# xiaochuanle/hifimeth

Hardware: AMD Instinct MI355X
Metric: cytosine sites/sec (CpG+CHG+CHH) (higher is better)
Workload: dtype f16x3+f32acc

## Files before the change

### hifimeth_amd/csrc/hm_convs.h

```cpp
#pragma once
#include "hm_convh.h"

namespace hm {

struct WRegs {
    half8 w[12][4][2];
    float4 bz[4];
};

struct DenseRows {
    static constexpr bool DENSE = true;
    static constexpr int M = 1 << 30;
};
template <int LOUT, int ISS, int MSTR, int ROW0, int M_>
struct SiteRows {
    static constexpr bool DENSE = false;
    static constexpr int M = M_;
    template <class C>
    static __device__ __forceinline__ int off(int m) {
        const int mc = m < M ? m : M - 1, site = mc / LOUT, p = mc - site * LOUT;
        return site * ISS + (MSTR * p + ROW0) * C::IRS;
    }
};

template <int CIN_, int KT_, int IRS_, int DIL_, bool WLO_, bool XLO_, int KSTACK_, int XD_, int NTW_ = 2>
struct SCfg {
    static constexpr int CIN = CIN_, KT = KT_, IRS = IRS_, DIL = DIL_, KSTACK = KSTACK_, XD = XD_, NTW = NTW_;
    static constexpr bool WLO = WLO_ && KSTACK_ == 0, XLO = XLO_;
    static constexpr int KB = KT * CIN / 32;
    static constexpr int WSTR = KSTACK ? 64 : 128;
    static constexpr int NTERM = 1 + (XLO ? 1 : 0) + (WLO ? 1 : 0);
    static_assert(KB <= 12 && (KT * CIN) % 32 == 0 && (CIN % 32 == 0 || KSTACK > 0), "bad streaming conv geometry");
    static __device__ __forceinline__ int lane_off(int kb, int lk) {
        if constexpr (KSTACK > 0) {
            int t = 4 * kb + lk;
            t = t >= 2 * KSTACK ? 0 : t >= KSTACK ? t - KSTACK : t;
            return t * IRS;
        } else {
            const int kk = kb * 32, tap = kk / CIN;
            return tap * DIL * IRS + (kk - tap * CIN) + 8 * lk;
        }
    }
};

template <int I, int N, class F>
__device__ __forceinline__ void static_for(F&& f) {
    if constexpr (I < N) {
        f(std::integral_constant<int, I>{});
        static_for<I + 1, N>(f);
    }
}

template <class C, int K0, int K1>
__device__ __forceinline__ void sconv_load_w(const half_t* __restrict__ wfrag, int nt0, int lane, WRegs& W) {
    const half8* wp = reinterpret_cast<const half8*>(wfrag) + (size_t)nt0 * C::KB * C::WSTR + lane;
    static_for<K0, K1>([&](auto kb_) __attribute__((always_inline)) {
        constexpr int kb = decltype(kb_)::value;
#pragma unroll
        for (int j = 0; j < C::NTW; ++j) {
            W.w[kb][j][0] = wp[(size_t)(j * C::KB + kb) * C::WSTR];
            if (C::WLO) W.w[kb][j][1] = wp[(size_t)(j * C::KB + kb) * C::WSTR + 64];
        }
    });
}
template <class C>
__device__ __forceinline__ void sconv_load_bias(const float* __restrict__ bias, int nt0, int lane, WRegs& W) {
#pragma unroll
    for (int j = 0; j < C::NTW; ++j) W.bz[j] = *reinterpret_cast<const float4*>(bias + (nt0 + j) * 16 + 4 * (lane >> 4));
}

template <class C, class CN, class RM, int T0, int... GS>
struct SConvR {
    static constexpr int NG = sizeof...(GS);
    static constexpr int gs[NG] = {GS...};
    static constexpr int gmax() { int m = 0; for (int g = 0; g < NG; ++g) m = gs[g] > m ? gs[g] : m; return m; }
    static constexpr int gs_at(int g) { return g < NG ? gs[g < NG ? g : 0] : 0; }
    static constexpr int NTW = C::NTW;
    static constexpr int tile0(int g) { int t = T0; for (int i = 0; i < g; ++i) t += gs[i]; return t; }
    static constexpr int GMAX = gmax(), KB = C::KB, NB = NG * KB, XS = C::XD + 1;

    struct NoCopy {
        static constexpr int CS = 0, NWV = 4;
        const uint8_t* rows = nullptr;
        half_t* g = nullptr;
    };
    template <int J0 = 0, class Epi, class Copy = NoCopy>
    static __device__ __forceinline__ void run(const half_t* __restrict__ in_hi, const half_t* __restrict__ in_lo, WRegs& W,
                                               Epi epi, const half_t* __restrict__ wnext, const float* __restrict__ bnext,
                                               int nt0, int nt0n, Copy cp = Copy{}, RM rm = RM{}) {
        int tid = threadIdx.x;
        asm volatile("" : "+v"(tid));
        const int lane = tid & 63, li = lane & 15, lk = lane >> 4;
        const int a0 = li * C::IRS;
        constexpr int NTILES = tile0(NG) - T0;
        int aoff[RM::DENSE ? 1 : NTILES];
        if constexpr (!RM::DENSE) {
#pragma unroll
            for (int t = 0; t < NTILES; ++t) aoff[t] = rm.template off<C>((T0 + t) * 16 + li);
        }
        f32x4 acc[2][GMAX][NTW];
        half8 x[XS][GMAX][2];
        constexpr int CS = Copy::CS;
        static_assert(CS + 2 <= NB, "a copy slot per k-block");
        int crow[3];
        half8 cdat[2];
        const uint8_t* cpr = CS > 0 ? cp.rows + 2 * __builtin_amdgcn_readfirstlane(tid >> 6) + (lane >> 5) : nullptr;

        auto reads = [&](auto c_) __attribute__((always_inline)) {
            constexpr int c = decltype(c_)::value, g = c / KB, kb = c % KB;
            const int off = C::lane_off(kb, lk);
#pragma unroll
            for (int i = 0; i < gs[g]; ++i) {
                int o;
                if constexpr (RM::DENSE) o = a0 + off + (tile0(g) + i) * 16 * C::IRS;
                else o = aoff[RM::DENSE ? 0 : tile0(g) + i - T0] + off;
                x[c % XS][i][0] = *reinterpret_cast<const half8*>(in_hi + o);
                if (C::XLO) x[c % XS][i][1] = *reinterpret_cast<const half8*>(in_lo + o);
            }
        };
        static_for<0, (C::XD < NB ? C::XD : NB)>(reads);

        static_for<0, NB>([&](auto c_) __attribute__((always_inline)) {
            constexpr int c = decltype(c_)::value, g = c / KB, kb = c % KB, G = gs[g];
            if constexpr (kb == 0) {
#pragma unroll
                for (int i = 0; i < G; ++i)
#pragma unroll
                    for (int j = 0; j < NTW; ++j) acc[g & 1][i][j] = f32x4{W.bz[J0 + j].x, W.bz[J0 + j].y, W.bz[J0 + j].z, W.bz[J0 + j].w};
            }
            if constexpr (!std::is_void_v<CN> && g == NG - 1 && kb == 0)
                sconv_load_bias<std::conditional_t<std::is_void_v<CN>, C, CN>>(bnext, nt0n, lane, W);
            if constexpr (c + C::XD < NB) reads(std::integral_constant<int, c + C::XD>{});
#pragma unroll
            for (int pr = 0; pr < 3; ++pr) {
                if ((pr == 1 && !C::XLO) || (pr == 2 && !C::WLO)) continue;
#pragma unroll
                for (int i = 0; i < G; ++i)
#pragma unroll
                    for (int j = 0; j < NTW; ++j)
                        acc[g & 1][i][j] = __builtin_amdgcn_mfma_f32_16x16x32_f16(W.w[kb][J0 + j][pr == 2 ? 1 : 0], x[c % XS][i][pr == 1 ? 1 : 0],
                                                                                 acc[g & 1][i][j], 0, 0, 0);
            }
            constexpr int NA = g > 0 ? gs[g > 0 ? g - 1 : 0] * NTW : 0;
            constexpr int A0 = kb * NA / KB, A1 = (kb + 1) * NA / KB;
            if constexpr (g > 0) {
#pragma unroll
                for (int a = A0; a < A1; ++a) {
                    const int m = (tile0(g - 1) + a / NTW) * 16 + li;
                    if ((tile0(g - 1) + a / NTW + 1) * 16 <= RM::M || m < RM::M) epi(m, (nt0 + J0 + a % NTW) * 16 + 4 * lk, acc[(g - 1) & 1][a / NTW][a % NTW]);
                }
            }
            if constexpr (c >= 2 && c < CS + 2)
                *reinterpret_cast<half8*>(cp.g + (size_t)crow[(c - 2) % 3] * 256 + (lane & 31) * 8) = cdat[(c - 2) & 1];
            if constexpr (c >= 1 && c < CS + 1)
                cdat[(c - 1) & 1] = *reinterpret_cast<const half8*>(((lane & 16) ? in_lo : in_hi) + crow[(c - 1) % 3] * C::IRS + (lane & 15) * 8);
            if constexpr (c < CS) crow[c % 3] = cpr[c * 2 * Copy::NWV];
            if constexpr (!std::is_void_v<CN>) {
                using CNN = std::conditional_t<std::is_void_v<CN>, C, CN>;
                constexpr int NPN = CNN::WLO ? 2 : 1, EN = CNN::KB * CNN::NTW * NPN;
                auto is_free = [](int e) constexpr {
                    const int kb2 = e / (CNN::NTW * NPN), j2 = e / NPN % CNN::NTW, p2 = e % NPN;
                    return kb2 >= KB || j2 < J0 || j2 >= J0 + NTW || p2 >= (C::WLO ? 2 : 1);
                };
                constexpr int NFREE = [&]() constexpr { int n = 0; for (int e = 0; e < EN; ++e) n += is_free(e); return n; }();
                constexpr int NEARLY = NB - KB;
                const half8* wp = reinterpret_cast<const half8*>(wnext) + (size_t)nt0n * CNN::KB * CNN::WSTR + lane;
                static_for<0, EN>([&](auto e_) __attribute__((always_inline)) {
                    constexpr int e = decltype(e_)::value;
                    constexpr int kb2 = e / (CNN::NTW * NPN), j2 = e / NPN % CNN::NTW, p2 = e % NPN;
                    constexpr bool fr = is_free(e);
                    constexpr int rank = [&]() constexpr { int n = 0; for (int q = 0; q < e; ++q) n += is_free(q); return n; }();
                    constexpr bool now = fr ? (NEARLY > 0 ? (c < NEARLY && rank * NEARLY / (NFREE > 0 ? NFREE : 1) == c) : (c == NB - KB))
                                            : (g == NG - 1 && kb2 == kb);
                    if constexpr (now) W.w[kb2][j2][p2] = wp[(size_t)(j2 * CNN::KB + kb2) * CNN::WSTR + 64 * p2];
                });
            }
            {
                constexpr int ND = gs_at((c + C::XD) / KB) * (C::XLO ? 2 : 1);
                constexpr int NM = C::NTERM * G * NTW;
                constexpr int NR = NM > ND ? NM - ND : 1;
                constexpr int NV = g > 0 ? ((A1 - A0) * 24 + NR - 1) / NR : 0;
#pragma unroll
                for (int q = 0; q < (ND < NM ? ND : NM); ++q) {
                    __builtin_amdgcn_sched_group_barrier(0x008, 1, 0);
                    __builtin_amdgcn_sched_group_barrier(0x100, 1, 0);
                }
#pragma unroll
                for (int q = 0; q < NM - ND; ++q) {
                    __builtin_amdgcn_sched_group_barrier(0x008, 1, 0);
                    if (NV > 0) __builtin_amdgcn_sched_group_barrier(0x002, NV, 0);
                    if (NV > 0) __builtin_amdgcn_sched_group_barrier(0x200, 1, 0);
                    __builtin_amdgcn_sched_group_barrier(0x020, 1, 0);
                    if (c <= CS + 1) __builtin_amdgcn_sched_group_barrier(0x140, 1, 0);
                }
            }
            __builtin_amdgcn_sched_barrier(0);
        });
        {
            constexpr int g = NG - 1;
#pragma unroll
            for (int a = 0; a < gs[g] * NTW; ++a) {
                const int m = (tile0(g) + a / NTW) * 16 + li;
                if ((tile0(g) + a / NTW + 1) * 16 <= RM::M || m < RM::M) epi(m, (nt0 + J0 + a % NTW) * 16 + 4 * lk, acc[g & 1][a / NTW][a % NTW]);
            }
        }
    }
};

template <class C, class CN, int T0, int... GS>
using SConv = SConvR<C, CN, DenseRows, T0, GS...>;

}
```

### hifimeth_amd/csrc/hm_trunk3.hip

```cpp
#include "hm_convh.h"
#ifdef HM_TRUNK_STAMP
#include "hm_stamp.h"
namespace hm { __device__ unsigned long long g_trunk3_stamp[8][24]; }
extern "C" int hm_debug_trunk3_stamps(unsigned long long* out, int reset) {
    if (out && hipMemcpyFromSymbol(out, HIP_SYMBOL(hm::g_trunk3_stamp), sizeof(hm::g_trunk3_stamp)) != hipSuccess) return -1;
    if (reset) {
        static unsigned long long z[8][24];
        if (hipMemcpyToSymbol(HIP_SYMBOL(hm::g_trunk3_stamp), z, sizeof(z)) != hipSuccess) return -1;
    }
    return 0;
}
#endif
#include "hm_convs.h"
#include "hm_edge.h"

namespace hm {

namespace {

constexpr int T3_M = TR_OWN;
constexpr int T3_H1 = 4, T3_H2 = 8, T3_H3 = 16;
constexpr int T3_S3 = T3_H3, T3_S2 = T3_S3 + T3_H2, T3_S1 = T3_S2 + T3_H1;
constexpr int T3_AROWS = T3_M + T3_H3, T3_BROWS = T3_M + T3_H2;
constexpr int T3_XROWS = 128;
constexpr int T3_LDS_HALVES = 2 * T3_AROWS * TR_RS + 2 * T3_BROWS * TR_RS + 2 * (T3_H1 + T3_H3) * TR_RS;
constexpr int T3_N4 = 64, T3_RL3 = 3 * TR_OWN, T3_RL = T3_RL3 + T3_N4 + 4;
constexpr int T3_RLW = 3 * 32 + T3_N4 / 4 + 1;
static_assert(T3_M % 16 == 0 && T3_RL % 4 == 0 && T3_RL / 4 <= 256 && T3_XROWS >= T3_M + 12, "tile plan");

struct ListRows4 {
    static constexpr bool DENSE = false;
    static constexpr int M = T3_N4;
    const uint8_t* rows = nullptr;
    template <class C>
    __device__ __forceinline__ int off(int m) const { return (int)rows[m] * C::IRS; }
};
struct EpiE4L {
    half_t* __restrict__ g;
    const uint8_t* rows;
    __device__ __forceinline__ void operator()(int m, int col, const f32x4& acc) const {
        half4 h, l;
        split4(acc, h, l);
        const size_t o = (size_t)rows[m] * (2 * C4_CH) + col;
        *reinterpret_cast<half4*>(g + o) = h;
        *reinterpret_cast<half4*>(g + o + C4_CH) = l;
    }
};

struct EpiTrunk3 {
    half_t* hi;
    half_t* lo;
    __device__ __forceinline__ void operator()(int m, int col, const f32x4& acc) const {
        half4 h, l;
        split4(acc, h, l);
        *reinterpret_cast<half4*>(hi + m * TR_RS + col) = h;
        *reinterpret_cast<half4*>(lo + m * TR_RS + col) = l;
    }
};
struct EpiE43 {
    half_t* __restrict__ g;
    __device__ __forceinline__ void operator()(int m, int col, const f32x4& acc) const {
        half4 h, l;
        split4(acc, h, l);
        *reinterpret_cast<half4*>(g + (size_t)m * (2 * C4_CH) + col) = h;
        *reinterpret_cast<half4*>(g + (size_t)m * (2 * C4_CH) + C4_CH + col) = l;
    }
};
template <int NWV_>
struct CopyRows3 {
    static constexpr int NWV = NWV_, CS = TR_OWN / (2 * NWV_);
    const uint8_t* rows;
    half_t* g;
};

__device__ __forceinline__ void t3_lds_barrier() {
    __builtin_amdgcn_fence(__ATOMIC_RELEASE, "workgroup", "local");
    __builtin_amdgcn_s_barrier();
    __builtin_amdgcn_fence(__ATOMIC_ACQUIRE, "workgroup", "local");
}

template <int NROWS, int NT, int K = 0>
__device__ __forceinline__ void move_rows(half_t* dh, half_t* dl, const half_t* sh, const half_t* sl, int t) {
    constexpr int PER = NROWS * TR_RS / 8, N = 2 * PER;
    if constexpr (K * NT < N) {
        const int c = min(t + K * NT, N - 1), plane = c >= PER, o = (c - plane * PER) * 8;
        const uint4 v = *reinterpret_cast<const uint4*>((plane ? sl : sh) + o);
        move_rows<NROWS, NT, K + 1>(dh, dl, sh, sl, t);
        *reinterpret_cast<uint4*>((plane ? dl : dh) + o) = v;
    }
}

}

constexpr int T3_RPB = 4;
template <int K1>
__global__ __launch_bounds__(64) void rowlist3_kernel(const TrunkTile* __restrict__ tiles, int n_tiles, int n_work, int ctx,
                                                       const RInfo* __restrict__ rinfo, const uint8_t* __restrict__ sctx, int64_t n_bases,
                                                       uint8_t* __restrict__ rowlist) {
    using G = EdgeGeo<K1>;
    const int r = threadIdx.x;
    constexpr int first_new[3] = {T3_H1, T3_H2, T3_H3}, shift[3] = {T3_S1, T3_S2, T3_S3};
    constexpr int W0 = -176, WN = 528;
    __shared__ __attribute__((aligned(4))) uint8_t rec[T3_RPB][T3_RL];
    __shared__ __attribute__((aligned(4))) uint8_t sf[T3_RPB][WN];
    static_assert(-G::R1 - 2 + T3_S1 >= W0 && -G::R2 - 4 + T3_S2 >= W0 && -G::R3 - 8 + T3_S3 >= W0 && T3_S1 + TR_OWN - 1 - G::LEFT < W0 + WN &&
                  215 - 16 * 23 >= W0 && TR_OWN - 1 + 215 - 16 < W0 + WN, "the window covers every lookup");
    int kind[T3_RPB];
    TrunkTile tl[T3_RPB];
    RInfo ri[T3_RPB];
    bool warm[T3_RPB];
    int view[T3_RPB];
#pragma unroll
    for (int k = 0; k < T3_RPB; ++k) {
        const int blk = (int)blockIdx.x * T3_RPB + k;
        kind[k] = blk > 2 * n_work ? 0 : blk == 2 * n_work ? 2 : 1;
        warm[k] = blk >= n_work;
        const int w = min(warm[k] ? blk - n_work : blk, n_work - 1);
        view[k] = w >= n_tiles;
        tl[k] = tiles[view[k] ? w - n_tiles : w];
    }
    bool any = false;
#pragma unroll
    for (int k = 0; k < T3_RPB; ++k) {
        if (kind[k] == 1 && warm[k] && tl[k].u0 != -TR_PAD) kind[k] = 0;
        any |= kind[k] != 0;
    }
    if (!any) return;
#pragma unroll
    for (int k = 0; k < T3_RPB; ++k) ri[k] = rinfo[tl[k].read_idx];
    constexpr int NQ = (WN / 4 + 63) / 64;
    static_assert(WN % 4 == 0 && (-W0) % 4 == 0 && TR_PAD % 4 == 0 && TR_OWN % 4 == 0, "windows start on multiples of 4");
    uint32_t sw[T3_RPB][NQ];
#pragma unroll
    for (int k = 0; k < T3_RPB; ++k) {
        const int L = ri[k].len, u = tl[k].u0 - (warm[k] ? TR_OWN : 0);
#pragma unroll
        for (int q = 0; q < NQ; ++q) {
            const int y0 = u + W0 + 4 * (r + 64 * q);
            const int64_t a = view[k] ? ri[k].base_off + (L - 1 - y0 - 3) : ri[k].base_off + y0;
            if (a >= 0 && a + 4 <= n_bases) {
                uint32_t v;
                __builtin_memcpy(&v, sctx + a, 4);
                sw[k][q] = view[k] ? __builtin_bswap32(v) : v;
            } else {
                uint32_t v = 0;
#pragma unroll
                for (int t = 0; t < 4; ++t) {
                    const int64_t j = view[k] ? ri[k].base_off + (L - 1 - y0 - t) : ri[k].base_off + y0 + t;
                    v |= (uint32_t)(j >= 0 && j < n_bases ? sctx[j] : (uint8_t)CTX_NONE) << (8 * t);
                }
                sw[k][q] = v;
            }
        }
    }
#pragma unroll
    for (int k = 0; k < T3_RPB; ++k) {
        for (int i = r; i < T3_RL3; i += 64) rec[k][i] = (uint8_t)(first_new[i / TR_OWN] + TR_OWN - 1);
        const int L = ri[k].len, u = tl[k].u0 - (warm[k] ? TR_OWN : 0);
        const uint32_t key = (uint32_t)(ctx | (view[k] << 2)) * 0x01010101u;
#pragma unroll
        for (int q = 0; q < NQ; ++q) {
            const int y0 = u + W0 + 4 * (r + 64 * q);
            const uint32_t x = sw[k][q] ^ key;
            uint32_t hit = (~(((x & 0x7F7F7F7Fu) + 0x7F7F7F7Fu) | x | 0x7F7F7F7Fu)) >> 7;
            const int lo = min(max(-y0, 0), 4), hi = min(max(L - y0, 0), 4);
            const uint32_t m_hi = hi >= 4 ? 0xFFFFFFFFu : (1u << (8 * hi)) - 1u, m_lo = lo >= 4 ? 0xFFFFFFFFu : (1u << (8 * lo)) - 1u;
            hit &= m_hi & ~m_lo;
            if (r + 64 * q < WN / 4) reinterpret_cast<uint32_t*>(sf[k])[r + 64 * q] = hit;
        }
    }
    __syncthreads();
    const uint64_t below = (1ull << r) - 1;
#pragma unroll
    for (int k = 0; k < T3_RPB; ++k) {
        if (kind[k] == 0) continue;
        const int blk = (int)blockIdx.x * T3_RPB + k;
        int n4 = 255;
        if (kind[k] == 1) {
            const int u = tl[k].u0 - (warm[k] ? TR_OWN : 0);
            auto sat = [&](int y) __attribute__((always_inline)) { return (int)sf[k][y - u - W0]; };
            const bool want4 = K1 == 11 && !warm[k];
            int f[2] = {0, 0}, need4[2] = {0, 0};
#pragma unroll
            for (int h = 0; h < 2; ++h) {
                const int row = r + 64 * h;
                if (row < TR_OWN) {
                    {
                        const int x = u + shift[0] + row;
                        f[h] |= (sat(x - G::LEFT) | sat(x - G::R1) | (G::PAD2 ? 0 : sat(x - G::R1 - 2))) << 0;
                    }
                    {
                        const int x = u + shift[1] + row;
                        f[h] |= (sat(x - G::LEFT) | sat(x - G::R2) | (G::PAD3 ? 0 : sat(x - G::R2 - 4))) << 1;
                    }
                    {
                        const int x = u + shift[2] + row;
                        f[h] |= (sat(x - G::LEFT) | sat(x - G::R3) | (G::PAD4 ? 0 : sat(x - G::R3 - 8))) << 2;
                    }
                    if (want4) {
#pragma unroll
                        for (int sidx = 1; sidx <= 23; ++sidx) need4[h] |= sat(u + row + 215 - 16 * sidx);
                    }
                }
            }
#pragma unroll
            for (int l = 0; l < 3; ++l) {
                const uint64_t b0 = __ballot((f[0] >> l) & 1), b1 = __ballot((f[1] >> l) & 1);
                if ((f[0] >> l) & 1) rec[k][l * TR_OWN + __popcll(b0 & below)] = (uint8_t)(first_new[l] + r);
                if ((f[1] >> l) & 1) rec[k][l * TR_OWN + __popcll(b0) + __popcll(b1 & below)] = (uint8_t)(first_new[l] + r + 64);
            }
            const uint64_t n0 = __ballot(need4[0]), n1 = __ballot(need4[1]);
            if (want4) n4 = __popcll(n0) + __popcll(n1);
            if (want4 && n4 <= T3_N4) {
                if (need4[0]) rec[k][T3_RL3 + __popcll(n0 & below)] = (uint8_t)r;
                if (need4[1]) rec[k][T3_RL3 + __popcll(n0) + __popcll(n1 & below)] = (uint8_t)(r + 64);
                __syncthreads();
                if (r >= n4) rec[k][T3_RL3 + r] = n4 > 0 ? rec[k][T3_RL3] : (uint8_t)0;
            }
        }
        if (r == 0) *reinterpret_cast<uint32_t*>(&rec[k][T3_RL3 + T3_N4]) = (uint32_t)n4;
        __syncthreads();
        uint32_t* out = reinterpret_cast<uint32_t*>(rowlist + (size_t)blk * T3_RL);
        for (int i = r; i < T3_RL / 4; i += 64) out[i] = reinterpret_cast<const uint32_t*>(rec[k])[i];
    }
}

template <int K1, bool W3LO = true>
__global__ __launch_bounds__(256) __attribute__((amdgpu_waves_per_eu(1, 1)))
void trunk3_kernel(const TrunkTile* __restrict__ tiles, int n_tiles, int n_views, int ctx, const RInfo* __restrict__ rinfo,
                   const uint8_t* __restrict__ bases, const uint32_t* __restrict__ kin, CtxWeights W, TrunkMaps mp, half_t* __restrict__ dump,
                   int32_t* __restrict__ list_steps, const int32_t* __restrict__ tcost) {
    constexpr int NW = 4, NTW = 2;
    __shared__ __attribute__((aligned(16))) half_t smem[T3_LDS_HALVES + T3_XROWS * TR_WRS];
    static_assert(sizeof(smem) == 147840, "LDS plan");
    __shared__ uint32_t rlist[2][T3_RLW];
    __shared__ int64_t s_grow0;
    __shared__ int s_kind;
    __shared__ __attribute__((aligned(16))) half_t kc[3][2][128];
    __shared__ __attribute__((aligned(16))) half_t e4c[2 * C4_CH];
    half_t* a_hi = smem;
    half_t* a_lo = a_hi + T3_AROWS * TR_RS;
    half_t* b_hi = a_lo + T3_AROWS * TR_RS;
    half_t* b_lo = b_hi + T3_BROWS * TR_RS;
    half_t* h1_hi = b_lo + T3_BROWS * TR_RS;
    half_t* h1_lo = h1_hi + T3_H1 * TR_RS;
    half_t* h3_hi = h1_lo + T3_H1 * TR_RS;
    half_t* h3_lo = h3_hi + T3_H3 * TR_RS;
    half_t* xb = h3_lo + T3_H3 * TR_RS;
    const int n_work = n_tiles * n_views;
    const int lane = threadIdx.x & 63, wave = __builtin_amdgcn_readfirstlane(threadIdx.x >> 6);
    int w0, w1;
    if (tcost) {
        const int64_t c_view = tcost[n_tiles], c_all = c_view * n_views;
        auto cost_at = [&](const int wq) __attribute__((always_inline)) {
            const int v = wq >= n_tiles && wq < n_work ? 1 : wq >= n_work ? n_views : 0;
            return v * c_view + (wq >= n_work ? 0 : tcost[wq - (v ? n_tiles : 0)]);
        };
        auto first_at = [&](const int64_t target) __attribute__((always_inline)) {
            int lo = 0, hi = n_work;
            while (hi > lo) {
                const int stride = (hi - lo + 63) / 64;
                const int probe = lo + lane * stride;
                const bool ge = probe >= hi || cost_at(probe) >= target;
                const uint64_t bal = __ballot(ge);
                const int first = bal ? __builtin_ctzll(bal) : 64;
                if (first == 0) {
                    hi = lo;
                } else {
                    const int nlo = lo + (first - 1) * stride + 1;
                    hi = first < 64 ? min(lo + first * stride, hi) : hi;
                    lo = nlo;
                }
            }
            return __builtin_amdgcn_readfirstlane(lo);
        };
        const int64_t k = blockIdx.x, G = gridDim.x;
        w0 = first_at((k * c_all + G - 1) / G);
        w1 = k + 1 == G ? n_work : first_at(((k + 1) * c_all + G - 1) / G);
    } else {
        const int base_n = n_work / (int)gridDim.x, rem_n = n_work - base_n * (int)gridDim.x;
        w0 = (int)blockIdx.x * base_n + min((int)blockIdx.x, rem_n);
        w1 = w0 + base_n + ((int)blockIdx.x < rem_n);
    }
    if (w0 >= w1) return;

    for (int i = threadIdx.x; i < (T3_LDS_HALVES + T3_XROWS * TR_WRS) / 2; i += NW * 64) reinterpret_cast<uint32_t*>(smem)[i] = 0u;
    for (int i = threadIdx.x; i < 2 * T3_RLW; i += NW * 64) rlist[0][i] = 0;
    __syncthreads();

    struct Build {
        TrunkTile tl, tl2;
        RInfo ri;
        int w, view, warm, cst, calib, ueff, b;
        uint32_t k, rl;
    } bd;
    auto build_desc1 = [&](const int w) __attribute__((always_inline)) {
        bd.w = w;
        bd.view = w >= n_tiles;
        bd.tl = tiles[bd.view ? w - n_tiles : w];
        const int w2 = min(w + 1, n_work - 1);
        bd.tl2 = tiles[w2 >= n_tiles ? w2 - n_tiles : w2];
    };
    auto build_desc2 = [&](const int prev_warm, const bool first) __attribute__((always_inline)) {
        bd.tl.read_idx = __builtin_amdgcn_readfirstlane(bd.tl.read_idx);
        bd.tl.u0 = __builtin_amdgcn_readfirstlane(bd.tl.u0);
        bd.warm = first ? 1 : (prev_warm ? 0 : (bd.tl.u0 == -TR_PAD));
        bd.calib = 0;
        bd.ueff = bd.tl.u0 - (bd.warm ? TR_OWN : 0);
        bd.ri = rinfo[bd.tl.read_idx];
    };
    auto build_desc3 = [&]() __attribute__((always_inline)) {
        bd.ri.len = __builtin_amdgcn_readfirstlane(bd.ri.len);
        bd.ri.map_off = __builtin_amdgcn_readfirstlane(bd.ri.map_off);
        bd.ri.base_off = ((int64_t)__builtin_amdgcn_readfirstlane((int)(bd.ri.base_off >> 32)) << 32) |
                         (uint32_t)__builtin_amdgcn_readfirstlane((int)bd.ri.base_off);
        bd.cst = bd.tl.u0 == -TR_PAD || (!bd.warm && bd.tl.u0 >= bd.ri.len);
    };
    auto build_loads = [&]() __attribute__((always_inline)) {
        const int r = threadIdx.x, L = bd.ri.len, x = bd.ueff + T3_S1 + r;
        const int xc = min(max(x, 0), L - 1);
        const int64_t j = bd.ri.base_off + (bd.view ? L - 1 - xc : xc);
        bd.b = bases[j];
        bd.k = kin[j];
        const size_t li = bd.calib ? (size_t)2 * n_work : bd.warm ? (bd.tl.u0 == -TR_PAD ? (size_t)n_work + bd.w : (size_t)2 * n_work) : (size_t)bd.w;
        bd.rl = reinterpret_cast<const uint32_t*>(mp.rowlist + li * T3_RL)[min(r, T3_RL / 4 - 1)];
    };
    auto build_store = [&](const int buf) __attribute__((always_inline)) {
        const int r = threadIdx.x, x = bd.ueff + T3_S1 + r;
        if (r == 0) {
            s_grow0 = (int64_t)bd.view * mp.view_rows + bd.ri.map_off + (bd.ueff + TR_PAD);
            s_kind = bd.warm | (bd.cst << 1) | (bd.calib << 2);
        }
        if (r < T3_XROWS) {
            const bool in = !bd.calib && x >= 0 && x < bd.ri.len;
            *reinterpret_cast<uint4*>(xb + r * TR_WRS) = feature_row(in ? bd.b : -1, bd.k, bd.view);
        }
        if (r < T3_RL3 / 4) rlist[buf][r / (TR_OWN / 4) * 32 + r % (TR_OWN / 4)] = bd.rl;
        else if (r < T3_RL / 4) rlist[buf][3 * 32 + r - T3_RL3 / 4] = bd.rl;
    };

    using C1 = SCfg<8, (2 * K1 + 3) / 4 * 4, TR_WRS, 1, true, false, K1, 2, NTW>;
    using C2 = SCfg<128, 3, TR_RS, 2, true, true, 0, 1, NTW>;
    using C3 = SCfg<128, 3, TR_RS, 4, W3LO, true, 0, 1, NTW>;
    using C4 = SCfg<128, 3, TR_RS, 8, true, true, 0, 1, NTW>;
    using C4s = SCfg<128, 3, TR_RS, 8, true, true, 0, 1, 1>;
    const int nt04 = wave == 0 ? 0 : wave == 1 ? 1 : wave == 2 ? 3 : 4;
    using L1 = SConv<C1, C2, 0, 2, 2, 3>;
    using L2 = SConv<C2, C3, 0, 3, 4>;
    using L3 = SConv<C3, C4, 0, 3, 4>;
    static_assert(T3_XROWS <= NW * 64, "one feature row per thread");
    auto wf = [&](int i) { return reinterpret_cast<const half_t*>(W.wfrag_h[i]); };
    const half_t* c1f = reinterpret_cast<const half_t*>(W.c1f);
    const int nt0 = NTW * wave;

    WRegs wr;
    sconv_load_w<C1, 0, C1::KB>(c1f, nt0, lane, wr);
    sconv_load_bias<C1>(W.c1f_bias, nt0, lane, wr);
    build_desc1(w0);
    build_desc2(0, true);
    build_desc3();
    bd.calib = 1;
    bd.cst = 0;
    build_loads();
    build_store(0);
    int buf = 0;
    int w = w0, warm = 1;
    int n_list = 0;
    int n_const = 0;
    bool prev_calib = false;
    half_t* const dump_rows = dump + TR_OWN * 2 * C4_CH;
    half_t* const dump_cal = dump_rows + 128 * 256 + (size_t)blockIdx.x * (TR_OWN * 2 * C4_CH);
    constexpr int first_new[3] = {T3_H1, T3_H2, T3_H3};
#ifdef HM_TRUNK_STAMP
    unsigned long long ts[10], acc_t[16] = {};
    unsigned long long n_it = 0, acc_c = 0, n_c = 0;
    const bool st_on = blockIdx.x == 0;
    const unsigned long long tk0 = hm_stamp(), tr0 = __builtin_amdgcn_s_memrealtime();
#define TS(i) do { if (st_on) ts[i] = hm_stamp(); } while (0)
#else
#define TS(i)
#endif
    while (true) {
        t3_lds_barrier();
        TS(0);
        const int64_t grow0 = s_grow0;
        const int kind = __builtin_amdgcn_readfirstlane(s_kind);
        const int cur_warm = kind & 1, cur_const = (kind >> 1) & 1, cur_calib = kind >> 2;
        if (prev_calib) {
            prev_calib = false;
            __builtin_amdgcn_fence(__ATOMIC_ACQUIRE, "agent");
            const int t = threadIdx.x;
            if (t < 96) {
                const int l = t >> 5, plane = (t >> 4) & 1, col = (t & 15) * 8;
                const half_t* src = l == 0 ? (plane ? h1_lo : h1_hi) : l == 1 ? (plane ? b_lo : b_hi) : (plane ? h3_lo : h3_hi);
                *reinterpret_cast<uint4*>(&kc[l][plane][col]) = *reinterpret_cast<const uint4*>(src + col);
            } else if (t < 96 + 24) {
                reinterpret_cast<uint4*>(e4c)[t - 96] = reinterpret_cast<const uint4*>(dump_cal + (TR_OWN - 1) * 2 * C4_CH)[t - 96];
            }
            __syncthreads();
        }
        const int wn = cur_warm ? w : w + 1;
        const bool last = wn >= w1;
        half_t* g1 = cur_calib ? dump_rows : reinterpret_cast<half_t*>(mp.e[0]) + (grow0 + T3_S2) * 256;
        half_t* g2 = cur_calib ? dump_rows : reinterpret_cast<half_t*>(mp.e[1]) + (grow0 + T3_S3) * 256;
        half_t* g3 = cur_calib ? dump_rows : reinterpret_cast<half_t*>(mp.e[2]) + grow0 * 256;
        const uint8_t* rl = reinterpret_cast<const uint8_t*>(rlist[buf]);
        if (cur_const) {
            const int t = threadIdx.x;
            n_const += !cur_warm;
            const int wb = min(wn, w1 - 1);
            bool new_read = false;
            if (wb != bd.w) {
                const int prev_read = bd.tl.read_idx;
                bd.w = wb;
                bd.view = wb >= n_tiles;
                bd.tl.read_idx = __builtin_amdgcn_readfirstlane(bd.tl2.read_idx);
                bd.tl.u0 = __builtin_amdgcn_readfirstlane(bd.tl2.u0);
                const int w2 = min(wb + 1, n_work - 1);
                bd.tl2 = tiles[w2 >= n_tiles ? w2 - n_tiles : w2];
                new_read = bd.tl.read_idx != prev_read;
                if (new_read) bd.ri = rinfo[bd.tl.read_idx];
            }
            auto finish_desc = [&]() __attribute__((always_inline)) {
                bd.warm = cur_warm ? 0 : (bd.tl.u0 == -TR_PAD);
                bd.calib = 0;
                bd.ueff = bd.tl.u0 - (bd.warm ? TR_OWN : 0);
                bd.cst = bd.tl.u0 == -TR_PAD || (!bd.warm && bd.tl.u0 >= bd.ri.len);
                build_loads();
            };
            if (!new_read) finish_desc();
            if (!cur_warm) {
                uint4* g4 = reinterpret_cast<uint4*>(reinterpret_cast<half_t*>(mp.e4) + grow0 * (2 * C4_CH));
                const uint4 v = reinterpret_cast<const uint4*>(e4c)[t % 24];
                const uint4 v2 = reinterpret_cast<const uint4*>(e4c)[(t + 16) % 24], v3 = reinterpret_cast<const uint4*>(e4c)[(t + 8) % 24];
#pragma unroll
                for (int k = 0; k < (TR_OWN * 24 + 255) / 256; ++k) {
                    const int c = t + 256 * k;
                    if (c < TR_OWN * 24) g4[c] = k % 3 == 0 ? v : k % 3 == 1 ? v2 : v3;
                }
            }
#pragma unroll
            for (int l = 0; l < 3; ++l) {
                const uint8_t* rows = rl + 128 * l;
                half_t* g = l == 0 ? g1 : l == 1 ? g2 : g3;
                const int fill = first_new[l] + TR_OWN - 1, ch = t & 31;
                const uint4 v = reinterpret_cast<const uint4*>(&kc[l][0][0])[ch];
                int pr[TR_OWN / 8];
#pragma unroll
                for (int i = 0; i < TR_OWN / 8; ++i) pr[i] = rows[(t >> 5) + 8 * i];
#pragma unroll
                for (int i = 0; i < TR_OWN / 8; ++i)
                    if (pr[i] != fill) reinterpret_cast<uint4*>(g + (size_t)pr[i] * 256)[ch] = v;
                if (t < 32) reinterpret_cast<uint4*>(g + (size_t)fill * 256)[ch] = v;
            }
            for (int c = t; c < (T3_H1 + T3_H2 + T3_H3) * 32; c += NW * 64) {
                const int row = c >> 5, plane = (c >> 4) & 1, col = (c & 15) * 8;
                const int l = row < T3_H1 ? 0 : row < T3_H1 + T3_H2 ? 1 : 2, r = row - (l == 0 ? 0 : l == 1 ? T3_H1 : T3_H1 + T3_H2);
                half_t* dst = (l == 0 ? (plane ? h1_lo : h1_hi) : l == 1 ? (plane ? b_lo : b_hi) : (plane ? h3_lo : h3_hi)) + r * TR_RS + col;
                *reinterpret_cast<uint4*>(dst) = *reinterpret_cast<const uint4*>(&kc[l][plane][col]);
            }
            if (new_read) {
                build_desc3();
                finish_desc();
            }
            t3_lds_barrier();
            build_store(buf ^ 1);
            buf ^= 1;
#ifdef HM_TRUNK_STAMP
            if (st_on) {
                acc_c += hm_stamp() - ts[0];
                ++n_c;
            }
#endif
            if (last) break;
            w = wn;
            warm = bd.warm;
            continue;
        }
        move_rows<T3_H1, NW * 64>(a_hi, a_lo, h1_hi, h1_lo, threadIdx.x);
        L1::run(xb, xb, wr, EpiTrunk3{a_hi + T3_H1 * TR_RS, a_lo + T3_H1 * TR_RS}, wf(1), W.bias[1], nt0, nt0);
        build_desc1(min(wn, w1 - 1));
        TS(1);
        __syncthreads();
        TS(2);
        build_desc2(cur_warm, cur_calib != 0);
        L2::run(a_hi, a_lo, wr, EpiTrunk3{b_hi + T3_H2 * TR_RS, b_lo + T3_H2 * TR_RS}, wf(2), W.bias[2], nt0, nt0, CopyRows3<NW>{rl, g1});
        move_rows<T3_H1, NW * 64>(h1_hi, h1_lo, a_hi + T3_M * TR_RS, a_lo + T3_M * TR_RS, threadIdx.x);
        TS(3);
        __syncthreads();
        TS(4);
        build_desc3();
        build_loads();
        move_rows<T3_H3, NW * 64>(a_hi, a_lo, h3_hi, h3_lo, threadIdx.x);
        L3::run(b_hi, b_lo, wr, EpiTrunk3{a_hi + T3_H3 * TR_RS, a_lo + T3_H3 * TR_RS}, wf(3), W.bias[3], nt0, nt04, CopyRows3<NW>{rl + 128, g2});
        TS(5);
        __syncthreads();
        TS(6);
        move_rows<T3_H3, NW * 64>(h3_hi, h3_lo, a_hi + T3_M * TR_RS, a_lo + T3_M * TR_RS, threadIdx.x);
        move_rows<T3_H2, NW * 64>(b_hi, b_lo, b_hi + T3_M * TR_RS, b_lo + T3_M * TR_RS, threadIdx.x);
        const EpiE43 e4{cur_calib ? dump_cal : cur_warm ? dump : reinterpret_cast<half_t*>(mp.e4) + grow0 * (2 * C4_CH)};
        const int n4 = __builtin_amdgcn_readfirstlane((int)rlist[buf][T3_RLW - 1]);
        if (!cur_warm && n4 <= T3_N4) {
            ++n_list;
            const uint8_t* rows4 = rl + 3 * 128;
            const ListRows4 rm{rows4};
            const EpiE4L e4l{reinterpret_cast<half_t*>(mp.e4) + grow0 * (2 * C4_CH), rows4};
            using NoCp = typename SConvR<C4, C1, ListRows4, 2, 2>::NoCopy;
            if (wave & 1) {
                SConvR<C4s, void, ListRows4, 0, 1, 1>::template run<1>(a_hi, a_lo, wr, e4l, c1f, W.c1f_bias, nt04, nt0, CopyRows3<NW>{rl + 256, g3}, rm);
                SConvR<C4, C1, ListRows4, 2, 2>::run(a_hi, a_lo, wr, e4l, c1f, W.c1f_bias, nt04, nt0, NoCp{}, rm);
            } else {
                SConvR<C4, void, ListRows4, 0, 1, 1>::run(a_hi, a_lo, wr, e4l, c1f, W.c1f_bias, nt04, nt0, CopyRows3<NW>{rl + 256, g3}, rm);
                SConvR<C4s, C1, ListRows4, 2, 2>::template run<0>(a_hi, a_lo, wr, e4l, c1f, W.c1f_bias, nt04, nt0, NoCp{}, rm);
            }
        } else
        if (wave & 1) {
            SConv<C4s, void, 0, 2, 2>::template run<1>(a_hi, a_lo, wr, e4, c1f, W.c1f_bias, nt04, nt0, CopyRows3<NW>{rl + 256, g3});
            SConv<C4, C1, 4, 3>::run(a_hi, a_lo, wr, e4, c1f, W.c1f_bias, nt04, nt0);
        } else {
            SConv<C4, void, 0, 2, 2>::run(a_hi, a_lo, wr, e4, c1f, W.c1f_bias, nt04, nt0, CopyRows3<NW>{rl + 256, g3});
            SConv<C4s, C1, 4, 3>::template run<0>(a_hi, a_lo, wr, e4, c1f, W.c1f_bias, nt04, nt0);
        }
        build_store(buf ^ 1);
        buf ^= 1;
        if (cur_calib) {
            __builtin_amdgcn_fence(__ATOMIC_RELEASE, "agent");
            prev_calib = true;
        }
        TS(7);
#ifdef HM_TRUNK_STAMP
        if (st_on) {
            __syncthreads();
            ts[8] = hm_stamp();
            for (int l = 0; l < 4; ++l) {
                acc_t[4 * l + 0] += ts[2 * l + 1] - ts[2 * l];
                acc_t[4 * l + 3] += ts[2 * l + 2] - ts[2 * l + 1];
            }
            ++n_it;
        }
#endif
        if (last) break;
        w = wn;
        warm = bd.warm;
    }
    (void)warm;
#ifdef HM_TRUNK_STAMP
    if (st_on && (threadIdx.x & 63) == 0) {
        for (int i = 0; i < 16; ++i) atomicAdd(&g_trunk3_stamp[threadIdx.x >> 6][i], acc_t[i]);
        atomicAdd(&g_trunk3_stamp[threadIdx.x >> 6][16], n_it);
        atomicAdd(&g_trunk3_stamp[threadIdx.x >> 6][17], acc_c);
        atomicAdd(&g_trunk3_stamp[threadIdx.x >> 6][18], n_c);
        atomicAdd(&g_trunk3_stamp[threadIdx.x >> 6][22], hm_stamp() - tk0);
        atomicAdd(&g_trunk3_stamp[threadIdx.x >> 6][23], __builtin_amdgcn_s_memrealtime() - tr0);
    }
#endif
#undef TS
    if (list_steps && threadIdx.x == 0 && n_list) atomicAdd(list_steps + ctx, n_list);
    if (list_steps && threadIdx.x == 0 && n_const) atomicAdd(list_steps + 4 + ctx, n_const);
}

size_t trunk3_rowlist_bytes(int64_t n_work) { return (size_t)(2 * n_work + 1) * T3_RL + 64; }
size_t trunk3_dump_bytes(int grid) { return ((size_t)(1 + grid) * TR_OWN * 2 * C4_CH + 128 * 256) * sizeof(uint16_t); }

void launch_trunk3(hipStream_t st, int k1, const TrunkTile* tiles, int n_tiles, int n_views, int ctx, const RInfo* rinfo,
                   const uint8_t* bases, const uint32_t* kin, const uint8_t* sctx, int64_t n_bases, const CtxWeights& w, const TrunkMaps& maps,
                   uint16_t* dump, int32_t* list_steps, const int32_t* tcost, int grid, bool w3_single) {
    if (n_tiles <= 0) return;
    const int n_work = n_tiles * n_views;
    const dim3 g(min(n_work, grid));
    if (k1 == 11) {
        hipLaunchKernelGGL(rowlist3_kernel<11>, dim3((2 * n_work + T3_RPB) / T3_RPB), dim3(64), 0, st, tiles, n_tiles, n_work, ctx, rinfo, sctx, n_bases, maps.rowlist);
        if (w3_single) hipLaunchKernelGGL((trunk3_kernel<11, false>), g, dim3(256), 0, st, tiles, n_tiles, n_views, ctx, rinfo, bases, kin, w, maps, reinterpret_cast<half_t*>(dump), list_steps, tcost);
        else hipLaunchKernelGGL((trunk3_kernel<11, true>), g, dim3(256), 0, st, tiles, n_tiles, n_views, ctx, rinfo, bases, kin, w, maps, reinterpret_cast<half_t*>(dump), list_steps, tcost);
    } else {
        hipLaunchKernelGGL(rowlist3_kernel<13>, dim3((2 * n_work + T3_RPB) / T3_RPB), dim3(64), 0, st, tiles, n_tiles, n_work, ctx, rinfo, sctx, n_bases, maps.rowlist);
        if (w3_single) hipLaunchKernelGGL((trunk3_kernel<13, false>), g, dim3(256), 0, st, tiles, n_tiles, n_views, ctx, rinfo, bases, kin, w, maps, reinterpret_cast<half_t*>(dump), list_steps, tcost);
        else hipLaunchKernelGGL((trunk3_kernel<13, true>), g, dim3(256), 0, st, tiles, n_tiles, n_views, ctx, rinfo, bases, kin, w, maps, reinterpret_cast<half_t*>(dump), list_steps, tcost);
    }
}

}
```

Before: 68.25 million.

## Specialize interleaved row-copy slots by per-tile copy count and regroup L2/L3 tiles

The row-list builder now also packs the number of rows each layer actually needs to copy into the descriptor word. The conv kernels use this count to pick, at runtime, one of several compile-time tiers (2, 4, 6 or all slots) of interleaved global copy instructions. This lets tiles with few rows to copy skip most of the copy work hidden in the MFMA loop. L2 and L3 also move from a 3+4 tile grouping to 2+2+3, giving the head blocks room for the tiered copies. The cost is several specialized code paths, which grows code size and instruction-cache pressure and changes the schedule.

```diff
diff --git a/hifimeth_amd/csrc/hm_convs.h b/hifimeth_amd/csrc/hm_convs.h
--- a/hifimeth_amd/csrc/hm_convs.h
+++ b/hifimeth_amd/csrc/hm_convs.h
@@ -43,6 +43,17 @@
     }
 };
 
+template <class T, class = void>
+struct copy_is_tiered : std::false_type {
+    static constexpr int NT = 0;
+    static constexpr int tier(int) { return 0; }
+};
+template <class T>
+struct copy_is_tiered<T, std::enable_if_t<T::TIERED>> : std::true_type {
+    static constexpr int NT = T::NT;
+    static constexpr int tier(int i) { return T::tier(i); }
+};
+
 template <int I, int N, class F>
 __device__ __forceinline__ void static_for(F&& f) {
     if constexpr (I < N) {
@@ -102,6 +113,9 @@
         half8 x[XS][GMAX][2];
         constexpr int CS = Copy::CS;
         static_assert(CS + 2 <= NB, "a copy slot per k-block");
+        constexpr bool TIERED = copy_is_tiered<Copy>::value;
+        constexpr int NHEAD = TIERED ? NB - KB : 0;
+        static_assert(!TIERED || (NG > 1 && CS + 2 <= NHEAD), "a tiered copy's slots end before the last group");
         int crow[3];
         half8 cdat[2];
         const uint8_t* cpr = CS > 0 ? cp.rows + 2 * __builtin_amdgcn_readfirstlane(tid >> 6) + (lane >> 5) : nullptr;
@@ -120,8 +134,9 @@
         };
         static_for<0, (C::XD < NB ? C::XD : NB)>(reads);
 
-        static_for<0, NB>([&](auto c_) __attribute__((always_inline)) {
+        auto block = [&](auto c_, auto cs_) __attribute__((always_inline)) {
             constexpr int c = decltype(c_)::value, g = c / KB, kb = c % KB, G = gs[g];
+            constexpr int CS = decltype(cs_)::value;
             if constexpr (kb == 0) {
 #pragma unroll
                 for (int i = 0; i < G; ++i)
@@ -195,7 +210,23 @@
                 }
             }
             __builtin_amdgcn_sched_barrier(0);
-        });
+        };
+        using CsAll = std::integral_constant<int, CS>;
+        if constexpr (TIERED) {
+            auto pick = [&](auto self, auto i_) __attribute__((always_inline)) -> void {
+                constexpr int i = decltype(i_)::value;
+                if constexpr (i == copy_is_tiered<Copy>::NT) {
+                    static_for<0, NHEAD>([&](auto c_) __attribute__((always_inline)) { block(c_, CsAll{}); });
+                } else {
+                    using CsI = std::integral_constant<int, copy_is_tiered<Copy>::tier(i)>;
+                    static_assert(CsI::value < CS, "short tiers in ascending order");
+                    if (cp.need <= 2 * Copy::NWV * CsI::value) static_for<0, NHEAD>([&](auto c_) __attribute__((always_inline)) { block(c_, CsI{}); });
+                    else self(self, std::integral_constant<int, i + 1>{});
+                }
+            };
+            pick(pick, std::integral_constant<int, 0>{});
+        }
+        static_for<NHEAD, NB>([&](auto c_) __attribute__((always_inline)) { block(c_, CsAll{}); });
         {
             constexpr int g = NG - 1;
 #pragma unroll
diff --git a/hifimeth_amd/csrc/hm_trunk3.hip b/hifimeth_amd/csrc/hm_trunk3.hip
--- a/hifimeth_amd/csrc/hm_trunk3.hip
+++ b/hifimeth_amd/csrc/hm_trunk3.hip
@@ -26,6 +26,8 @@
 constexpr int T3_LDS_HALVES = 2 * T3_AROWS * TR_RS + 2 * T3_BROWS * TR_RS + 2 * (T3_H1 + T3_H3) * TR_RS;
 constexpr int T3_N4 = 64, T3_RL3 = 3 * TR_OWN, T3_RL = T3_RL3 + T3_N4 + 4;
 constexpr int T3_RLW = 3 * 32 + T3_N4 / 4 + 1;
+constexpr int T3_TIER[] = {2, 4, 6};
+constexpr int T3_NT = sizeof(T3_TIER) / sizeof(int), T3_CS_ALL = TR_OWN / 8;
 static_assert(T3_M % 16 == 0 && T3_RL % 4 == 0 && T3_RL / 4 <= 256 && T3_XROWS >= T3_M + 12, "tile plan");
 
 struct ListRows4 {
@@ -66,11 +68,19 @@
         *reinterpret_cast<half4*>(g + (size_t)m * (2 * C4_CH) + C4_CH + col) = l;
     }
 };
-template <int NWV_>
+template <int NWV_, int CS_ = TR_OWN / (2 * NWV_)>
 struct CopyRows3 {
-    static constexpr int NWV = NWV_, CS = TR_OWN / (2 * NWV_);
+    static constexpr int NWV = NWV_, CS = CS_;
+    static_assert(CS_ >= 0 && 2 * NWV_ * CS_ <= TR_OWN, "slots within the list");
     const uint8_t* rows;
     half_t* g;
+};
+template <int NWV_>
+struct CopyRows3T : CopyRows3<NWV_> {
+    static constexpr bool TIERED = true;
+    static constexpr int NT = T3_NT;
+    static constexpr int tier(int i) { return T3_TIER[i]; }
+    int need;
 };
 
 __device__ __forceinline__ void t3_lds_barrier() {
@@ -176,6 +186,7 @@
         if (kind[k] == 0) continue;
         const int blk = (int)blockIdx.x * T3_RPB + k;
         int n4 = 255;
+        uint32_t nst = 0;
         if (kind[k] == 1) {
             const int u = tl[k].u0 - (warm[k] ? TR_OWN : 0);
             auto sat = [&](int y) __attribute__((always_inline)) { return (int)sf[k][y - u - W0]; };
@@ -208,6 +219,7 @@
                 const uint64_t b0 = __ballot((f[0] >> l) & 1), b1 = __ballot((f[1] >> l) & 1);
                 if ((f[0] >> l) & 1) rec[k][l * TR_OWN + __popcll(b0 & below)] = (uint8_t)(first_new[l] + r);
                 if ((f[1] >> l) & 1) rec[k][l * TR_OWN + __popcll(b0) + __popcll(b1 & below)] = (uint8_t)(first_new[l] + r + 64);
+                nst |= (uint32_t)(__popcll(b0) + __popcll(b1) + (int)(~(b1 >> (TR_OWN - 1 - 64)) & 1)) << (8 * (l + 1));
             }
             const uint64_t n0 = __ballot(need4[0]), n1 = __ballot(need4[1]);
             if (want4) n4 = __popcll(n0) + __popcll(n1);
@@ -218,7 +230,7 @@
                 if (r >= n4) rec[k][T3_RL3 + r] = n4 > 0 ? rec[k][T3_RL3] : (uint8_t)0;
             }
         }
-        if (r == 0) *reinterpret_cast<uint32_t*>(&rec[k][T3_RL3 + T3_N4]) = (uint32_t)n4;
+        if (r == 0) *reinterpret_cast<uint32_t*>(&rec[k][T3_RL3 + T3_N4]) = (uint32_t)n4 | nst;
         __syncthreads();
         uint32_t* out = reinterpret_cast<uint32_t*>(rowlist + (size_t)blk * T3_RL);
         for (int i = r; i < T3_RL / 4; i += 64) out[i] = reinterpret_cast<const uint32_t*>(rec[k])[i];
@@ -346,8 +358,8 @@
     using C4s = SCfg<128, 3, TR_RS, 8, true, true, 0, 1, 1>;
     const int nt04 = wave == 0 ? 0 : wave == 1 ? 1 : wave == 2 ? 3 : 4;
     using L1 = SConv<C1, C2, 0, 2, 2, 3>;
-    using L2 = SConv<C2, C3, 0, 3, 4>;
-    using L3 = SConv<C3, C4, 0, 3, 4>;
+    using L2 = SConv<C2, C3, 0, 2, 2, 3>;
+    using L3 = SConv<C3, C4, 0, 2, 2, 3>;
     static_assert(T3_XROWS <= NW * 64, "one feature row per thread");
     auto wf = [&](int i) { return reinterpret_cast<const half_t*>(W.wfrag_h[i]); };
     const half_t* c1f = reinterpret_cast<const half_t*>(W.c1f);
@@ -477,6 +489,25 @@
             warm = bd.warm;
             continue;
         }
+#ifdef HM_XP_T3_NOCOPY
+        struct Cp23 : CopyRows3<NW, 0> { int need; };
+#else
+        using Cp23 = CopyRows3T<NW>;
+#endif
+        const uint32_t cw = (uint32_t)__builtin_amdgcn_readfirstlane((int)rlist[buf][T3_RLW - 1]);
+        auto with_slots = [&](const int need, auto&& f) __attribute__((always_inline)) {
+#ifdef HM_XP_T3_NOCOPY
+            f(std::integral_constant<int, 0>{});
+#else
+            auto pick = [&](auto self, auto i_) __attribute__((always_inline)) -> void {
+                constexpr int i = decltype(i_)::value;
+                if constexpr (i == T3_NT) f(std::integral_constant<int, T3_CS_ALL>{});
+                else if (need <= 8 * T3_TIER[i]) f(std::integral_constant<int, T3_TIER[i]>{});
+                else self(self, std::integral_constant<int, i + 1>{});
+            };
+            pick(pick, std::integral_constant<int, 0>{});
+#endif
+        };
         move_rows<T3_H1, NW * 64>(a_hi, a_lo, h1_hi, h1_lo, threadIdx.x);
         L1::run(xb, xb, wr, EpiTrunk3{a_hi + T3_H1 * TR_RS, a_lo + T3_H1 * TR_RS}, wf(1), W.bias[1], nt0, nt0);
         build_desc1(min(wn, w1 - 1));
@@ -484,7 +515,7 @@
         __syncthreads();
         TS(2);
         build_desc2(cur_warm, cur_calib != 0);
-        L2::run(a_hi, a_lo, wr, EpiTrunk3{b_hi + T3_H2 * TR_RS, b_lo + T3_H2 * TR_RS}, wf(2), W.bias[2], nt0, nt0, CopyRows3<NW>{rl, g1});
+        L2::run(a_hi, a_lo, wr, EpiTrunk3{b_hi + T3_H2 * TR_RS, b_lo + T3_H2 * TR_RS}, wf(2), W.bias[2], nt0, nt0, Cp23{{rl, g1}, (int)((cw >> 8) & 255)});
         move_rows<T3_H1, NW * 64>(h1_hi, h1_lo, a_hi + T3_M * TR_RS, a_lo + T3_M * TR_RS, threadIdx.x);
         TS(3);
         __syncthreads();
@@ -492,14 +523,14 @@
         build_desc3();
         build_loads();
         move_rows<T3_H3, NW * 64>(a_hi, a_lo, h3_hi, h3_lo, threadIdx.x);
-        L3::run(b_hi, b_lo, wr, EpiTrunk3{a_hi + T3_H3 * TR_RS, a_lo + T3_H3 * TR_RS}, wf(3), W.bias[3], nt0, nt04, CopyRows3<NW>{rl + 128, g2});
+        L3::run(b_hi, b_lo, wr, EpiTrunk3{a_hi + T3_H3 * TR_RS, a_lo + T3_H3 * TR_RS}, wf(3), W.bias[3], nt0, nt04, Cp23{{rl + 128, g2}, (int)((cw >> 16) & 255)});
         TS(5);
         __syncthreads();
         TS(6);
         move_rows<T3_H3, NW * 64>(h3_hi, h3_lo, a_hi + T3_M * TR_RS, a_lo + T3_M * TR_RS, threadIdx.x);
         move_rows<T3_H2, NW * 64>(b_hi, b_lo, b_hi + T3_M * TR_RS, b_lo + T3_M * TR_RS, threadIdx.x);
         const EpiE43 e4{cur_calib ? dump_cal : cur_warm ? dump : reinterpret_cast<half_t*>(mp.e4) + grow0 * (2 * C4_CH)};
-        const int n4 = __builtin_amdgcn_readfirstlane((int)rlist[buf][T3_RLW - 1]);
+        const int n4 = cw & 255, ns3 = cw >> 24;
         if (!cur_warm && n4 <= T3_N4) {
             ++n_list;
             const uint8_t* rows4 = rl + 3 * 128;
@@ -507,18 +538,26 @@
             const EpiE4L e4l{reinterpret_cast<half_t*>(mp.e4) + grow0 * (2 * C4_CH), rows4};
             using NoCp = typename SConvR<C4, C1, ListRows4, 2, 2>::NoCopy;
             if (wave & 1) {
-                SConvR<C4s, void, ListRows4, 0, 1, 1>::template run<1>(a_hi, a_lo, wr, e4l, c1f, W.c1f_bias, nt04, nt0, CopyRows3<NW>{rl + 256, g3}, rm);
+                with_slots(ns3, [&](auto cs_) __attribute__((always_inline)) {
+                    SConvR<C4s, void, ListRows4, 0, 1, 1>::template run<1>(a_hi, a_lo, wr, e4l, c1f, W.c1f_bias, nt04, nt0, CopyRows3<NW, decltype(cs_)::value>{rl + 256, g3}, rm);
+                });
                 SConvR<C4, C1, ListRows4, 2, 2>::run(a_hi, a_lo, wr, e4l, c1f, W.c1f_bias, nt04, nt0, NoCp{}, rm);
             } else {
-                SConvR<C4, void, ListRows4, 0, 1, 1>::run(a_hi, a_lo, wr, e4l, c1f, W.c1f_bias, nt04, nt0, CopyRows3<NW>{rl + 256, g3}, rm);
+                with_slots(ns3, [&](auto cs_) __attribute__((always_inline)) {
+                    SConvR<C4, void, ListRows4, 0, 1, 1>::run(a_hi, a_lo, wr, e4l, c1f, W.c1f_bias, nt04, nt0, CopyRows3<NW, decltype(cs_)::value>{rl + 256, g3}, rm);
+                });
                 SConvR<C4s, C1, ListRows4, 2, 2>::template run<0>(a_hi, a_lo, wr, e4l, c1f, W.c1f_bias, nt04, nt0, NoCp{}, rm);
             }
         } else
         if (wave & 1) {
-            SConv<C4s, void, 0, 2, 2>::template run<1>(a_hi, a_lo, wr, e4, c1f, W.c1f_bias, nt04, nt0, CopyRows3<NW>{rl + 256, g3});
+            with_slots(ns3, [&](auto cs_) __attribute__((always_inline)) {
+                SConv<C4s, void, 0, 2, 2>::template run<1>(a_hi, a_lo, wr, e4, c1f, W.c1f_bias, nt04, nt0, CopyRows3<NW, decltype(cs_)::value>{rl + 256, g3});
+            });
             SConv<C4, C1, 4, 3>::run(a_hi, a_lo, wr, e4, c1f, W.c1f_bias, nt04, nt0);
         } else {
-            SConv<C4, void, 0, 2, 2>::run(a_hi, a_lo, wr, e4, c1f, W.c1f_bias, nt04, nt0, CopyRows3<NW>{rl + 256, g3});
+            with_slots(ns3, [&](auto cs_) __attribute__((always_inline)) {
+                SConv<C4, void, 0, 2, 2>::run(a_hi, a_lo, wr, e4, c1f, W.c1f_bias, nt04, nt0, CopyRows3<NW, decltype(cs_)::value>{rl + 256, g3});
+            });
             SConv<C4s, C1, 4, 3>::template run<0>(a_hi, a_lo, wr, e4, c1f, W.c1f_bias, nt04, nt0);
         }
         build_store(buf ^ 1);
```

Result: faster. 69.00 million (median of 6 runs) (+1.1%).
